# AUTOMATIC1111/stable-diffusion-webui

Measured on NVIDIA H100. Metric: images/sec SD1.5 txt2img 512x512, 20 Euler-a steps, batch 8 per GPU, higher is better.
Workload: dtype bf16

## Files before the change

### stable-diffusion-webui_b200/csrc/common.cuh

```cuda
#pragma once
#include <cuda.h>
#include <cuda_runtime.h>
#include <cuda_fp16.h>
#include <cuda_bf16.h>
#include <stdint.h>
#include <cstdio>
#include <cstring>

namespace sdxe {

enum : int { DT_F16 = 0, DT_BF16 = 1, DT_F32 = 2 };

#define SDXE_DEVINL __device__ __forceinline__

SDXE_DEVINL uint32_t smem_u32(const void* p) { return (uint32_t)__cvta_generic_to_shared(p); }
SDXE_DEVINL uint32_t lane_id() { return threadIdx.x & 31; }

SDXE_DEVINL bool elect_one() {
  uint32_t pred = 0;
  asm volatile(
      "{\n\t.reg .b32 rx;\n\t.reg .pred px;\n\t"
      "elect.sync rx|px, 0xffffffff;\n\t"
      "selp.b32 %0, 1, 0, px;\n\t}\n"
      : "=r"(pred));
  return pred != 0;
}

SDXE_DEVINL void mbar_init(uint32_t bar, uint32_t count) {
  asm volatile("mbarrier.init.shared::cta.b64 [%0], %1;" ::"r"(bar), "r"(count) : "memory");
}
SDXE_DEVINL void fence_mbar_init() { asm volatile("fence.mbarrier_init.release.cluster;" ::: "memory"); }
SDXE_DEVINL void mbar_expect_tx(uint32_t bar, uint32_t bytes) {
  asm volatile("mbarrier.arrive.expect_tx.shared::cta.b64 _, [%0], %1;" ::"r"(bar), "r"(bytes) : "memory");
}
SDXE_DEVINL void mbar_arrive(uint32_t bar) {
  asm volatile("mbarrier.arrive.shared::cta.b64 _, [%0];" ::"r"(bar) : "memory");
}
SDXE_DEVINL uint64_t global_timer_ns() {
  uint64_t t;
  asm volatile("mov.u64 %0, %%globaltimer;" : "=l"(t));
  return t;
}
SDXE_DEVINL void mbar_wait(uint32_t bar, uint32_t parity) {
  uint32_t done = 0;
  uint64_t t0 = 0;
  for (uint32_t it = 0;; ++it) {
    asm volatile(
        "{\n\t.reg .pred p;\n\t"
        "mbarrier.try_wait.parity.shared::cta.b64 p, [%1], %2;\n\t"
        "selp.b32 %0, 1, 0, p;\n\t}\n"
        : "=r"(done)
        : "r"(bar), "r"(parity)
        : "memory");
    if (done) return;
    if ((it & 0x3ff) == 0x3ff) {
      uint64_t now = global_timer_ns();
      if (t0 == 0) t0 = now;
      else if (now - t0 > 4000000000ull) __trap();
    }
  }
}

SDXE_DEVINL void pdl_launch_dependents() { asm volatile("griddepcontrol.launch_dependents;" ::: "memory"); }
SDXE_DEVINL void pdl_wait() { asm volatile("griddepcontrol.wait;" ::: "memory"); }

SDXE_DEVINL bool mbar_test(uint32_t bar, uint32_t parity) {
  uint32_t done;
  asm volatile(
      "{\n\t.reg .pred p;\n\t"
      "mbarrier.test_wait.parity.shared::cta.b64 p, [%1], %2;\n\t"
      "selp.b32 %0, 1, 0, p;\n\t}\n"
      : "=r"(done)
      : "r"(bar), "r"(parity)
      : "memory");
  return done != 0;
}

SDXE_DEVINL void fence_proxy_async_smem() { asm volatile("fence.proxy.async.shared::cta;" ::: "memory"); }

SDXE_DEVINL void tma_prefetch_desc(const CUtensorMap* m) {
  asm volatile("prefetch.tensormap [%0];" ::"l"(reinterpret_cast<uint64_t>(m)) : "memory");
}
SDXE_DEVINL void tma_load_2d(uint32_t dst, const CUtensorMap* m, uint32_t bar, int c0, int c1) {
  asm volatile(
      "cp.async.bulk.tensor.2d.shared::cluster.global.mbarrier::complete_tx::bytes [%0], [%1, {%3, %4}], [%2];"
      ::"r"(dst), "l"(reinterpret_cast<uint64_t>(m)), "r"(bar), "r"(c0), "r"(c1)
      : "memory");
}
SDXE_DEVINL void tma_load_3d(uint32_t dst, const CUtensorMap* m, uint32_t bar, int c0, int c1, int c2) {
  asm volatile(
      "cp.async.bulk.tensor.3d.shared::cluster.global.mbarrier::complete_tx::bytes [%0], [%1, {%3, %4, %5}], [%2];"
      ::"r"(dst), "l"(reinterpret_cast<uint64_t>(m)), "r"(bar), "r"(c0), "r"(c1), "r"(c2)
      : "memory");
}
SDXE_DEVINL void tma_load_4d(uint32_t dst, const CUtensorMap* m, uint32_t bar, int c0, int c1, int c2, int c3) {
  asm volatile(
      "cp.async.bulk.tensor.4d.shared::cluster.global.mbarrier::complete_tx::bytes [%0], [%1, {%3, %4, %5, %6}], [%2];"
      ::"r"(dst), "l"(reinterpret_cast<uint64_t>(m)), "r"(bar), "r"(c0), "r"(c1), "r"(c2), "r"(c3)
      : "memory");
}
SDXE_DEVINL void tma_load_5d(uint32_t dst, const CUtensorMap* m, uint32_t bar, int c0, int c1, int c2, int c3, int c4) {
  asm volatile(
      "cp.async.bulk.tensor.5d.shared::cluster.global.mbarrier::complete_tx::bytes [%0], [%1, {%3, %4, %5, %6, %7}], [%2];"
      ::"r"(dst), "l"(reinterpret_cast<uint64_t>(m)), "r"(bar), "r"(c0), "r"(c1), "r"(c2), "r"(c3), "r"(c4)
      : "memory");
}

SDXE_DEVINL void tma_store_2d(const CUtensorMap* m, uint32_t src, int c0, int c1) {
  asm volatile("cp.async.bulk.tensor.2d.global.shared::cta.bulk_group [%0, {%2, %3}], [%1];"
               ::"l"(reinterpret_cast<uint64_t>(m)), "r"(src), "r"(c0), "r"(c1)
               : "memory");
}
SDXE_DEVINL void bulk_commit_group() { asm volatile("cp.async.bulk.commit_group;" ::: "memory"); }
SDXE_DEVINL void bulk_wait_read_all() { asm volatile("cp.async.bulk.wait_group.read 0;" ::: "memory"); }
SDXE_DEVINL void bulk_wait_read_1() { asm volatile("cp.async.bulk.wait_group.read 1;" ::: "memory"); }
SDXE_DEVINL void bulk_wait_all() { asm volatile("cp.async.bulk.wait_group 0;" ::: "memory"); }

SDXE_DEVINL void wgmma_fence() { asm volatile("wgmma.fence.sync.aligned;" ::: "memory"); }
SDXE_DEVINL void wgmma_commit() { asm volatile("wgmma.commit_group.sync.aligned;" ::: "memory"); }
template <int N> SDXE_DEVINL void wgmma_wait() { asm volatile("wgmma.wait_group.sync.aligned %0;" ::"n"(N) : "memory"); }
SDXE_DEVINL void reg_fence(float& r) { asm volatile("" : "+f"(r)::"memory"); }

SDXE_DEVINL uint64_t gmma_desc_sw128(uint32_t saddr, uint32_t lbo_bytes, uint32_t sbo_bytes) {
  uint64_t d = 0;
  d |= (uint64_t)((saddr >> 4) & 0x3fff);
  d |= (uint64_t)((lbo_bytes >> 4) & 0x3fff) << 16;
  d |= (uint64_t)((sbo_bytes >> 4) & 0x3fff) << 32;
  d |= (uint64_t)1 << 62;
  return d;
}

template <bool BF16> struct T16;
template <> struct T16<false> {
  using type = __half;
  using type2 = __half2;
  static SDXE_DEVINL uint32_t pack(float a, float b) {
    __half2 h = __floats2half2_rn(a, b);
    return *reinterpret_cast<uint32_t*>(&h);
  }
  static SDXE_DEVINL float2 unpack(uint32_t u) { return __half22float2(*reinterpret_cast<__half2*>(&u)); }
  static SDXE_DEVINL float to_f(type v) { return __half2float(v); }
  static SDXE_DEVINL type from_f(float v) { return __float2half_rn(v); }
};
template <> struct T16<true> {
  using type = __nv_bfloat16;
  using type2 = __nv_bfloat162;
  static SDXE_DEVINL uint32_t pack(float a, float b) {
    __nv_bfloat162 h = __floats2bfloat162_rn(a, b);
    return *reinterpret_cast<uint32_t*>(&h);
  }
  static SDXE_DEVINL float2 unpack(uint32_t u) { return __bfloat1622float2(*reinterpret_cast<__nv_bfloat162*>(&u)); }
  static SDXE_DEVINL float to_f(type v) { return __bfloat162float(v); }
  static SDXE_DEVINL type from_f(float v) { return __float2bfloat16_rn(v); }
};

SDXE_DEVINL float ex2_approx(float x) {
  float y;
  asm("ex2.approx.ftz.f32 %0, %1;" : "=f"(y) : "f"(x));
  return y;
}
SDXE_DEVINL float ex2_poly3(float x) {
  x = fmaxf(x, -125.f);
  const float magic = 12582912.f;
  const float t = x + magic;
  const float r = x - (t - magic);
  float p = fmaf(0.0551716685295105f, r, 0.2426111400127411f);
  p = fmaf(p, r, 0.6932609677314758f);
  p = fmaf(p, r, 0.9999280571937561f);
  return __int_as_float(__float_as_int(p) + (__float_as_int(t) << 23));
}
SDXE_DEVINL float rcp_approx(float x) {
  float y;
  asm("rcp.approx.ftz.f32 %0, %1;" : "=f"(y) : "f"(x));
  return y;
}
SDXE_DEVINL float silu_f(float x) { return x * rcp_approx(1.f + ex2_approx(-1.4426950408889634f * x)); }
SDXE_DEVINL float gelu_erf_f(float x) { return 0.5f * x * (1.f + erff(x * 0.70710678118654752f)); }
#ifndef SDXE_GELU_V1
SDXE_DEVINL float gelu_fast_f(float x) {
  constexpr float C = 0.84932180028801904f;
  constexpr float S = 0.83255461115769776f;
  constexpr float H = 0.58870501125773735f;
  const float u = x * C;
  const float a = fabsf(u);
  const float t = rcp_approx(fmaf(0.3275911f * S, a, 1.f));
  float p = fmaf(1.061405429f * H, t, -1.453152027f * H);
  p = fmaf(p, t, 1.421413741f * H);
  p = fmaf(p, t, -0.284496736f * H);
  p = fmaf(p, t, 0.254829592f * H);
  const float e = ex2_approx(-u * u);
  return fmaf(-(a * e), p * t, fmaxf(x, 0.f));
}
#else
SDXE_DEVINL float gelu_fast_f(float x) {
  const float z = fabsf(x) * 0.70710678118654752f;
  const float t = rcp_approx(fmaf(0.3275911f, z, 1.f));
  float p = fmaf(1.061405429f, t, -1.453152027f);
  p = fmaf(p, t, 1.421413741f);
  p = fmaf(p, t, -0.284496736f);
  p = fmaf(p, t, 0.254829592f);
  const float e = ex2_approx(-z * z * 1.4426950408889634f);
  const float erf_abs = fmaf(-p * t, e, 1.f);
  const float erfv = copysignf(erf_abs, x);
  return 0.5f * x * (1.f + erfv);
}
#endif

#define SDXE_CUDA_CHECK(expr)                                                         \
  do {                                                                                \
    cudaError_t _e = (expr);                                                          \
    if (_e != cudaSuccess) {                                                          \
      ::sdxe::set_last_error(__FILE__, __LINE__, cudaGetErrorString(_e));             \
      return -1;                                                                      \
    }                                                                                 \
  } while (0)

void set_last_error(const char* file, int line, const char* msg);
const char* last_error();

int make_tmap_2d(CUtensorMap* out, const void* base, int64_t rows, int64_t cols, int64_t ld, int box_rows);
int make_tmap_2d_box(CUtensorMap* out, const void* base, int64_t rows, int64_t cols, int64_t ld, int box_cols, int box_rows);
int make_tmap_heads(CUtensorMap* out, const void* base, int64_t d, int64_t tokens, int64_t heads, int64_t batch,
                    int64_t tok_stride, int64_t head_stride, int64_t batch_stride, int box_rows);
int make_tmap_3d(CUtensorMap* out, const void* base, int64_t d0, int64_t d1, int64_t d2, int64_t pitch1, int64_t pitch2,
                 int box_rows);
int make_tmap_nhwc(CUtensorMap* out, const void* base, int N, int H, int W, int C, int bw, int bh, int bn);
int make_tmap_nhwc_s2(CUtensorMap* out, const void* base, int N, int H, int W, int C, int bw, int bh, int bn);

int num_sms();
bool pdl_enabled();

template <typename... KArgs, typename... Args>
inline cudaError_t launch_k(void (*kern)(KArgs...), dim3 grid, dim3 block, size_t smem, cudaStream_t s, Args&&... args) {
  cudaLaunchConfig_t cfg;
  memset(&cfg, 0, sizeof(cfg));
  cfg.gridDim = grid;
  cfg.blockDim = block;
  cfg.dynamicSmemBytes = smem;
  cfg.stream = s;
  cudaLaunchAttribute attr[1];
  attr[0].id = cudaLaunchAttributeProgrammaticStreamSerialization;
  attr[0].val.programmaticStreamSerializationAllowed = 1;
  cfg.attrs = attr;
  cfg.numAttrs = pdl_enabled() ? 1 : 0;
  return cudaLaunchKernelEx(&cfg, kern, static_cast<KArgs>(args)...);
}

}
```

### stable-diffusion-webui_b200/csrc/gemm.cu

```cuda
#include "gemm.cuh"
#include "wgmma.cuh"
#include <algorithm>
#include <cstdio>
#include <cstdlib>
#include <cstring>
#include <utility>

namespace sdxe {

static constexpr int BLOCK_M = 128;
static constexpr int BLOCK_K = 64;
static constexpr int A_STAGE_BYTES = BLOCK_M * BLOCK_K * 2;
static constexpr int GEMM_THREADS = 288;
static constexpr int CONSUMER_WARPS = 8;
static constexpr int SMEM_BUDGET = 227 * 1024;

template <int BN, bool BF16>
__global__ void __launch_bounds__(GEMM_THREADS, 1) gemm_kernel(const __grid_constant__ GemmArgs a) {
  using T = T16<BF16>;
  pdl_launch_dependents();
  extern __shared__ uint8_t smem_raw[];
  const uint32_t raw = smem_u32(smem_raw);
  const uint32_t smem_base = (raw + 1023u) & ~1023u;

  const int S = a.num_stages;
  constexpr uint32_t stage_bytes = A_STAGE_BYTES + BN * 128;
  const uint32_t bar_base = smem_base + S * stage_bytes;
  auto full_bar = [&](int s) { return bar_base + 8u * s; };
  auto empty_bar = [&](int s) { return bar_base + 8u * (S + s); };

  const int warp = threadIdx.x >> 5;
  const int lane = threadIdx.x & 31;
  const int num_m = (a.M + BLOCK_M - 1) / BLOCK_M;
  const int num_n = (a.N + BN - 1) / BN;
  const int num_kb = (a.K + BLOCK_K - 1) / BLOCK_K;
  const int num_tiles = num_m * num_n;

  if (threadIdx.x == 0) {
    for (int s = 0; s < S; ++s) {
      mbar_init(full_bar(s), 1);
      mbar_init(empty_bar(s), CONSUMER_WARPS);
    }
    fence_mbar_init();
    tma_prefetch_desc(&a.tmA);
    tma_prefetch_desc(&a.tmB);
  }
  __syncthreads();
  pdl_wait();

  if (warp == CONSUMER_WARPS) {
    int stage = 0;
    uint32_t phase = 0;
    for (int tile = blockIdx.x; tile < num_tiles; tile += gridDim.x) {
      const int n_blk = tile % num_n;
      const int m0 = (tile / num_n) * BLOCK_M;
      int img0 = 0, h0 = 0, w0 = 0;
      if (a.conv) {
        const int hw = a.H * a.W;
        img0 = m0 / hw;
        const int rem = m0 - img0 * hw;
        h0 = rem / a.W;
        w0 = rem - h0 * a.W;
      }
      int tap = 0, cb = 0;
      for (int kb = 0; kb < num_kb; ++kb) {
        mbar_wait(empty_bar(stage), phase ^ 1u);
        if (elect_one()) {
          const uint32_t sA = smem_base + stage * stage_bytes;
          const uint32_t sB = sA + A_STAGE_BYTES;
          const uint32_t fb = full_bar(stage);
          mbar_expect_tx(fb, stage_bytes);
          if (a.conv == 2) {
            const int dy = tap / 3, dx = tap - dy * 3;
            const int ty = dy - a.pad_lo, tx = dx - a.pad_lo;
            tma_load_5d(sA, &a.tmA, fb, (tx & 1) * (a.cblocks * BLOCK_K) + cb * BLOCK_K, w0 + (tx >> 1), ty & 1, h0 + (ty >> 1), img0);
          } else if (a.conv) {
            const int dy = tap / 3, dx = tap - dy * 3;
            tma_load_4d(sA, &a.tmA, fb, cb * BLOCK_K, w0 + dx - 1, h0 + dy - 1, img0);
          } else {
            const int k0 = kb * BLOCK_K;
            if (k0 < a.K1) tma_load_2d(sA, &a.tmA, fb, k0, m0);
            else tma_load_2d(sA, &a.tmA2, fb, k0 - a.K1, m0);
          }
          tma_load_2d(sB, &a.tmB, fb, kb * BLOCK_K, n_blk * BN);
        }
        __syncwarp();
        if (++cb == a.cblocks) { cb = 0; ++tap; }
        if (++stage == S) { stage = 0; phase ^= 1u; }
      }
    }
    return;
  }

  const int wg = warp >> 2;
  const int band = (warp & 3) * 16 + (lane >> 2);
  const int cq = 2 * (lane & 3);
  const int M = a.M, N = a.N;
  const uint64_t adesc0 = gmma_desc_sw128(smem_base + (uint32_t)wg * (64 * 128), 16, 1024);
  const uint64_t bdesc0 = gmma_desc_sw128(smem_base + A_STAGE_BYTES, 16, 1024);
  constexpr uint32_t stage_inc = stage_bytes >> 4;
  float acc[BN / 2];
  int stage = 0;
  uint32_t phase = 0;
  for (int tile = blockIdx.x; tile < num_tiles; tile += gridDim.x) {
    const int n_blk = tile % num_n;
    const int m_blk = tile / num_n;
    int prev = -1;
    for (int kb = 0; kb < num_kb; ++kb) {
      mbar_wait(full_bar(stage), phase);
      wgmma_fence();
      const uint64_t ad = adesc0 + (uint64_t)(stage * stage_inc);
      const uint64_t bd = bdesc0 + (uint64_t)(stage * stage_inc);
      wgmma_ss<BN, BF16>(acc, ad, bd, kb != 0);
      wgmma_ss<BN, BF16>(acc, ad + 2, bd + 2, 1);
      wgmma_ss<BN, BF16>(acc, ad + 4, bd + 4, 1);
      wgmma_ss<BN, BF16>(acc, ad + 6, bd + 6, 1);
      wgmma_commit();
      if (prev >= 0) {
        wgmma_wait<1>();
        if (lane == 0) mbar_arrive(empty_bar(prev));
      }
      prev = stage;
      if (++stage == S) { stage = 0; phase ^= 1u; }
    }
    wgmma_wait<0>();
#pragma unroll
    for (int i = 0; i < BN / 2; ++i) reg_fence(acc[i]);
    if (lane == 0 && prev >= 0) mbar_arrive(empty_bar(prev));

    const int row0 = m_blk * BLOCK_M + wg * 64 + band;
    float ln_mu[2] = {0.f, 0.f}, ln_rs[2] = {1.f, 1.f};
    if (a.c1) {
#pragma unroll
      for (int h = 0; h < 2; ++h) {
        const int m = row0 + 8 * h;
        float ps = 0.f, pq = 0.f;
        if (m < M) {
          for (int pp = 0; pp < a.ln_parts; ++pp) {
            const float2 t = __ldg(a.ln_part + (size_t)pp * M + m);
            ps += t.x;
            pq += t.y;
          }
        }
        ln_mu[h] = ps * a.ln_inv_c;
        ln_rs[h] = rsqrtf(fmaxf(pq * a.ln_inv_c - ln_mu[h] * ln_mu[h], 0.f) + a.ln_eps);
      }
    }
    if (a.epi == EPI_GEGLU) {
      constexpr int HALF = BN / 2;
      const int ldo = a.ldo;
#pragma unroll
      for (int i = 0; i < HALF / 8; ++i) {
        const int jl = 8 * i + cq;
        const int cv = n_blk * BN + jl, cg = cv + HALF;
        float bv[2] = {0.f, 0.f}, bg[2] = {0.f, 0.f}, kv[2] = {0.f, 0.f}, kg[2] = {0.f, 0.f};
        if (a.bias) { bv[0] = __ldg(a.bias + cv); bv[1] = __ldg(a.bias + cv + 1); bg[0] = __ldg(a.bias + cg); bg[1] = __ldg(a.bias + cg + 1); }
        if (a.c1) { kv[0] = __ldg(a.c1 + cv); kv[1] = __ldg(a.c1 + cv + 1); kg[0] = __ldg(a.c1 + cg); kg[1] = __ldg(a.c1 + cg + 1); }
#pragma unroll
        for (int h = 0; h < 2; ++h) {
          const int m = row0 + 8 * h;
          float o[2];
#pragma unroll
          for (int e = 0; e < 2; ++e) {
            float v = acc[4 * i + 2 * h + e], g = acc[4 * (i + HALF / 8) + 2 * h + e];
            if (a.c1) {
              v = fmaf(ln_rs[h], v - ln_mu[h] * kv[e], bv[e]);
              g = fmaf(ln_rs[h], g - ln_mu[h] * kg[e], bg[e]);
            } else {
              v += bv[e];
              g += bg[e];
            }
            o[e] = v * gelu_fast_f(g);
          }
          if (m < M) *reinterpret_cast<uint32_t*>(reinterpret_cast<uint16_t*>(a.out) + (size_t)m * ldo + n_blk * HALF + jl) = T::pack(o[0], o[1]);
        }
      }
    } else {
      const int n_store = std::min((N + 7) / 8 * 8, a.ldo);
      const int n_res = a.residual ? std::min((N + 7) / 8 * 8, a.ldr) : 0;
      const float* rv[2] = {nullptr, nullptr};
      bool row_ok[2];
#pragma unroll
      for (int h = 0; h < 2; ++h) {
        const int m = row0 + 8 * h;
        row_ok[h] = m < M;
        if (a.rowvec && row_ok[h]) rv[h] = a.rowvec + (size_t)(m / a.rows_per_sample) * a.ldrv;
      }
      float st_s[2] = {0.f, 0.f}, st_q[2] = {0.f, 0.f};
#pragma unroll
      for (int i = 0; i < BN / 8; ++i) {
        const int col = n_blk * BN + 8 * i + cq;
        if (col >= n_store) continue;
        const bool in0 = col < N, in1 = col + 1 < N;
        float b[2] = {0.f, 0.f}, k[2] = {0.f, 0.f};
        if (a.bias) { b[0] = in0 ? __ldg(a.bias + col) : 0.f; b[1] = in1 ? __ldg(a.bias + col + 1) : 0.f; }
        if (a.c1) { k[0] = in0 ? __ldg(a.c1 + col) : 0.f; k[1] = in1 ? __ldg(a.c1 + col + 1) : 0.f; }
#pragma unroll
        for (int h = 0; h < 2; ++h) {
          if (!row_ok[h]) continue;
          const size_t m = (size_t)(row0 + 8 * h);
          float v0 = acc[4 * i + 2 * h], v1 = acc[4 * i + 2 * h + 1];
          if (a.c1) {
            v0 = fmaf(ln_rs[h], v0 - ln_mu[h] * k[0], b[0]);
            v1 = fmaf(ln_rs[h], v1 - ln_mu[h] * k[1], b[1]);
          } else {
            v0 += b[0];
            v1 += b[1];
          }
          if (rv[h]) {
            if (in0) v0 += __ldg(rv[h] + col);
            if (in1) v1 += __ldg(rv[h] + col + 1);
          }
          if (col < n_res) {
            const uint32_t r = __ldg(reinterpret_cast<const unsigned int*>(reinterpret_cast<const uint16_t*>(a.residual) + m * a.ldr + col));
            const float2 f = T::unpack(r);
            v0 += f.x;
            v1 += f.y;
          }
          const uint32_t pk = T::pack(v0, v1);
          *reinterpret_cast<uint32_t*>(reinterpret_cast<uint16_t*>(a.out) + m * a.ldo + col) = pk;
          if (a.stat_out) {
            const float2 f = T::unpack(pk);
            const float x0 = in0 ? f.x : 0.f, x1 = in1 ? f.y : 0.f;
            st_s[h] += x0 + x1;
            st_q[h] = fmaf(x0, x0, fmaf(x1, x1, st_q[h]));
          }
        }
      }
      if (a.stat_out) {
#pragma unroll
        for (int h = 0; h < 2; ++h) {
          st_s[h] += __shfl_xor_sync(0xffffffffu, st_s[h], 1);
          st_q[h] += __shfl_xor_sync(0xffffffffu, st_q[h], 1);
          st_s[h] += __shfl_xor_sync(0xffffffffu, st_s[h], 2);
          st_q[h] += __shfl_xor_sync(0xffffffffu, st_q[h], 2);
          if ((lane & 3) == 0 && row_ok[h]) a.stat_out[(size_t)n_blk * M + row0 + 8 * h] = make_float2(st_s[h], st_q[h]);
        }
      }
    }
  }
}

bool conv_tile_shape(int H, int W, int* bw, int* bh, int* bn) {
  if (W >= 128) {
    if (W % 128) return false;
    *bw = 128; *bh = 1; *bn = 1;
    return true;
  }
  if (128 % W) return false;
  const int rows = 128 / W;
  if (H >= rows) {
    if (H % rows) return false;
    *bw = W; *bh = rows; *bn = 1;
    return true;
  }
  if (rows % H) return false;
  *bw = W; *bh = H; *bn = rows / H;
  return true;
}

static size_t gemm_smem_fixed(int num_stages) {
  return 1024  + 16 * (size_t)num_stages;
}
static size_t gemm_smem(int BN, int num_stages) { return (size_t)num_stages * (A_STAGE_BYTES + BN * 128) + gemm_smem_fixed(num_stages); }

int gemm_pick_stages(int BN) {
  const int stage_bytes = A_STAGE_BYTES + BN * 128;
  const int s = (int)((SMEM_BUDGET - gemm_smem_fixed(8)) / stage_bytes);
  return std::max(2, std::min(s, 8));
}

int gemm_finish_args(GemmArgs& a, const void* W, int64_t w_rows, int64_t w_ld) {
  a.num_stages = gemm_pick_stages(a.BN);
  if (a.ldo % 8 || (a.residual && a.ldr % 8)) { set_last_error(__FILE__, __LINE__, "gemm: ldo / ldr must be multiples of 8"); return -1; }
  return make_tmap_2d(&a.tmB, W, w_rows, a.K, w_ld, a.BN);
}

int gemm_pick_bn(int M, int N, int K, int epi) {
  (void)K;
  const int sms = num_sms();
  const int num_m = (M + BLOCK_M - 1) / BLOCK_M;
  double best = 1e30;
  int best_bn = 16;
  for (int bn = 16; bn <= 256; bn += 16) {
    if (epi == EPI_GEGLU && (bn % 32 != 0 || N % bn != 0)) continue;
    const int num_n = (N + bn - 1) / bn;
    const long tiles = (long)num_m * num_n;
    const long waves = (tiles + sms - 1) / sms;
    const double kb = std::max(4.0 * bn, (A_STAGE_BYTES + 128.0 * bn) / 32.0) + 64.0;
    const double cost = waves * kb;
    if (cost < best - 1e-9) { best = cost; best_bn = bn; }
  }
  return best_bn;
}

typedef void (*GemmKernel)(const GemmArgs);
static constexpr int GEMM_NUM_BN = 16;
template <std::size_t... I>
static GemmKernel gemm_variant_impl(int i, bool bf16, std::index_sequence<I...>) {
  static const GemmKernel k16[] = {gemm_kernel<16 * (int)(I + 1), false>...};
  static const GemmKernel kb16[] = {gemm_kernel<16 * (int)(I + 1), true>...};
  return bf16 ? kb16[i] : k16[i];
}
static GemmKernel gemm_variant(int BN, bool bf16) {
  return gemm_variant_impl(BN / 16 - 1, bf16, std::make_index_sequence<GEMM_NUM_BN>{});
}

int gemm_init() {
  static bool done = false;
  if (!done) {
    for (int bn = 16; bn <= 256; bn += 16)
      for (int b = 0; b < 2; ++b)
        SDXE_CUDA_CHECK(cudaFuncSetAttribute(gemm_variant(bn, b != 0), cudaFuncAttributeMaxDynamicSharedMemorySize, SMEM_BUDGET));
    done = true;
  }
  return 0;
}

int gemm_launch(const GemmArgs& a, bool bf16, cudaStream_t stream) {
  if (a.BN % 16 != 0 || a.BN < 16 || a.BN > 256) { set_last_error(__FILE__, __LINE__, "gemm: bad BN"); return -1; }
  if (a.K1 != a.K && (a.K1 % BLOCK_K) != 0) { set_last_error(__FILE__, __LINE__, "gemm: K1 % 64"); return -1; }
  if (a.epi == EPI_GEGLU && (a.BN % 32 != 0 || a.N % a.BN != 0)) { set_last_error(__FILE__, __LINE__, "gemm: geglu tile"); return -1; }
  if ((a.epi != EPI_PLAIN) && (a.residual || a.rowvec || a.stat_out)) { set_last_error(__FILE__, __LINE__, "gemm: residual / rowvec / statistics need EPI_PLAIN"); return -1; }
  if ((a.c1 && (a.residual || a.stat_out || a.rowvec)) || (a.stat_out && a.rowvec)) {
    set_last_error(__FILE__, __LINE__, "gemm: unsupported LayerNorm-fold / statistics combination");
    return -1;
  }
  if (a.num_stages < 2) { set_last_error(__FILE__, __LINE__, "gemm: stages (call gemm_finish_args)"); return -1; }
  const size_t smem = gemm_smem(a.BN, a.num_stages);
  if (smem > (size_t)SMEM_BUDGET) { set_last_error(__FILE__, __LINE__, "gemm: shared memory budget"); return -1; }
  const int num_m = (a.M + BLOCK_M - 1) / BLOCK_M, num_n = (a.N + a.BN - 1) / a.BN;
  const int tiles = num_m * num_n;
  if (tiles <= 0) return 0;
  if (gemm_init() != 0) return -1;
  const int grid = std::min(tiles, num_sms());
  SDXE_CUDA_CHECK(launch_k(gemm_variant(a.BN, bf16), dim3(grid), dim3(GEMM_THREADS), smem, stream, a));
  SDXE_CUDA_CHECK(cudaGetLastError());
  return 0;
}

}
```

Before: 8.499.

## Rebalance registers via setmaxnreg and batch epilogue loads in groups

Raises the block size to 384 threads (a full producer warpgroup) so setmaxnreg can move registers from producer warps (40) to consumer warps (232), and the three spare producer warps exit early. Separately, the GEMM epilogue now issues bias, LN-coefficient, row-vector and residual loads for groups of four column blocks before doing the arithmetic, so global-load latency overlaps instead of serializing per column. The intent is to ease register pressure from the large accumulator and hide epilogue load latency. The cost is more live registers in the epilogue and a dependency on setmaxnreg constraints, which require warpgroup-aligned launches and enough registers in the launch_bounds budget.

```diff
diff --git a/stable-diffusion-webui_b200/csrc/common.cuh b/stable-diffusion-webui_b200/csrc/common.cuh
--- a/stable-diffusion-webui_b200/csrc/common.cuh
+++ b/stable-diffusion-webui_b200/csrc/common.cuh
@@ -120,6 +120,9 @@
 SDXE_DEVINL void wgmma_commit() { asm volatile("wgmma.commit_group.sync.aligned;" ::: "memory"); }
 template <int N> SDXE_DEVINL void wgmma_wait() { asm volatile("wgmma.wait_group.sync.aligned %0;" ::"n"(N) : "memory"); }
 SDXE_DEVINL void reg_fence(float& r) { asm volatile("" : "+f"(r)::"memory"); }
+
+template <int N> SDXE_DEVINL void setmaxnreg_dec() { asm volatile("setmaxnreg.dec.sync.aligned.u32 %0;" ::"n"(N)); }
+template <int N> SDXE_DEVINL void setmaxnreg_inc() { asm volatile("setmaxnreg.inc.sync.aligned.u32 %0;" ::"n"(N)); }
 
 SDXE_DEVINL uint64_t gmma_desc_sw128(uint32_t saddr, uint32_t lbo_bytes, uint32_t sbo_bytes) {
   uint64_t d = 0;
diff --git a/stable-diffusion-webui_b200/csrc/gemm.cu b/stable-diffusion-webui_b200/csrc/gemm.cu
--- a/stable-diffusion-webui_b200/csrc/gemm.cu
+++ b/stable-diffusion-webui_b200/csrc/gemm.cu
@@ -11,8 +11,11 @@
 static constexpr int BLOCK_M = 128;
 static constexpr int BLOCK_K = 64;
 static constexpr int A_STAGE_BYTES = BLOCK_M * BLOCK_K * 2;
-static constexpr int GEMM_THREADS = 288;
+static constexpr int GEMM_THREADS = 384;
 static constexpr int CONSUMER_WARPS = 8;
+static constexpr int PRODUCER_REGS = 40;
+static constexpr int CONSUMER_REGS = 232;
+static constexpr int EPI_GROUPS = 4;
 static constexpr int SMEM_BUDGET = 227 * 1024;
 
 template <int BN, bool BF16>
@@ -48,7 +51,9 @@
   __syncthreads();
   pdl_wait();
 
-  if (warp == CONSUMER_WARPS) {
+  if (warp >= CONSUMER_WARPS) {
+    setmaxnreg_dec<PRODUCER_REGS>();
+    if (warp != CONSUMER_WARPS) return;
     int stage = 0;
     uint32_t phase = 0;
     for (int tile = blockIdx.x; tile < num_tiles; tile += gridDim.x) {
@@ -92,6 +97,7 @@
     return;
   }
 
+  setmaxnreg_inc<CONSUMER_REGS>();
   const int wg = warp >> 2;
   const int band = (warp & 3) * 16 + (lane >> 2);
   const int cq = 2 * (lane & 3);
@@ -150,80 +156,111 @@
       constexpr int HALF = BN / 2;
       const int ldo = a.ldo;
 #pragma unroll
-      for (int i = 0; i < HALF / 8; ++i) {
-        const int jl = 8 * i + cq;
-        const int cv = n_blk * BN + jl, cg = cv + HALF;
-        float bv[2] = {0.f, 0.f}, bg[2] = {0.f, 0.f}, kv[2] = {0.f, 0.f}, kg[2] = {0.f, 0.f};
-        if (a.bias) { bv[0] = __ldg(a.bias + cv); bv[1] = __ldg(a.bias + cv + 1); bg[0] = __ldg(a.bias + cg); bg[1] = __ldg(a.bias + cg + 1); }
-        if (a.c1) { kv[0] = __ldg(a.c1 + cv); kv[1] = __ldg(a.c1 + cv + 1); kg[0] = __ldg(a.c1 + cg); kg[1] = __ldg(a.c1 + cg + 1); }
-#pragma unroll
-        for (int h = 0; h < 2; ++h) {
-          const int m = row0 + 8 * h;
-          float o[2];
+      for (int i0 = 0; i0 < HALF / 8; i0 += EPI_GROUPS) {
+        float bv[EPI_GROUPS][2], bg[EPI_GROUPS][2], kv[EPI_GROUPS][2], kg[EPI_GROUPS][2];
+#pragma unroll
+        for (int g = 0; g < EPI_GROUPS && i0 + g < HALF / 8; ++g) {
+          const int cv = n_blk * BN + 8 * (i0 + g) + cq, cg = cv + HALF;
 #pragma unroll
           for (int e = 0; e < 2; ++e) {
-            float v = acc[4 * i + 2 * h + e], g = acc[4 * (i + HALF / 8) + 2 * h + e];
-            if (a.c1) {
-              v = fmaf(ln_rs[h], v - ln_mu[h] * kv[e], bv[e]);
-              g = fmaf(ln_rs[h], g - ln_mu[h] * kg[e], bg[e]);
-            } else {
-              v += bv[e];
-              g += bg[e];
-            }
-            o[e] = v * gelu_fast_f(g);
-          }
-          if (m < M) *reinterpret_cast<uint32_t*>(reinterpret_cast<uint16_t*>(a.out) + (size_t)m * ldo + n_blk * HALF + jl) = T::pack(o[0], o[1]);
+            bv[g][e] = a.bias ? __ldg(a.bias + cv + e) : 0.f;
+            bg[g][e] = a.bias ? __ldg(a.bias + cg + e) : 0.f;
+            kv[g][e] = a.c1 ? __ldg(a.c1 + cv + e) : 0.f;
+            kg[g][e] = a.c1 ? __ldg(a.c1 + cg + e) : 0.f;
+          }
+        }
+#pragma unroll
+        for (int g = 0; g < EPI_GROUPS && i0 + g < HALF / 8; ++g) {
+          const int i = i0 + g;
+          const int jl = 8 * i + cq;
+#pragma unroll
+          for (int h = 0; h < 2; ++h) {
+            const int m = row0 + 8 * h;
+            float o[2];
+#pragma unroll
+            for (int e = 0; e < 2; ++e) {
+              float v = acc[4 * i + 2 * h + e], gt = acc[4 * (i + HALF / 8) + 2 * h + e];
+              if (a.c1) {
+                v = fmaf(ln_rs[h], v - ln_mu[h] * kv[g][e], bv[g][e]);
+                gt = fmaf(ln_rs[h], gt - ln_mu[h] * kg[g][e], bg[g][e]);
+              } else {
+                v += bv[g][e];
+                gt += bg[g][e];
+              }
+              o[e] = v * gelu_fast_f(gt);
+            }
+            if (m < M) *reinterpret_cast<uint32_t*>(reinterpret_cast<uint16_t*>(a.out) + (size_t)m * ldo + n_blk * HALF + jl) = T::pack(o[0], o[1]);
+          }
         }
       }
     } else {
       const int n_store = std::min((N + 7) / 8 * 8, a.ldo);
       const int n_res = a.residual ? std::min((N + 7) / 8 * 8, a.ldr) : 0;
       const float* rv[2] = {nullptr, nullptr};
+      const uint16_t* rres[2] = {nullptr, nullptr};
       bool row_ok[2];
 #pragma unroll
       for (int h = 0; h < 2; ++h) {
         const int m = row0 + 8 * h;
         row_ok[h] = m < M;
         if (a.rowvec && row_ok[h]) rv[h] = a.rowvec + (size_t)(m / a.rows_per_sample) * a.ldrv;
+        if (a.residual && row_ok[h]) rres[h] = reinterpret_cast<const uint16_t*>(a.residual) + (size_t)m * a.ldr;
       }
       float st_s[2] = {0.f, 0.f}, st_q[2] = {0.f, 0.f};
 #pragma unroll
-      for (int i = 0; i < BN / 8; ++i) {
-        const int col = n_blk * BN + 8 * i + cq;
-        if (col >= n_store) continue;
-        const bool in0 = col < N, in1 = col + 1 < N;
-        float b[2] = {0.f, 0.f}, k[2] = {0.f, 0.f};
-        if (a.bias) { b[0] = in0 ? __ldg(a.bias + col) : 0.f; b[1] = in1 ? __ldg(a.bias + col + 1) : 0.f; }
-        if (a.c1) { k[0] = in0 ? __ldg(a.c1 + col) : 0.f; k[1] = in1 ? __ldg(a.c1 + col + 1) : 0.f; }
-#pragma unroll
-        for (int h = 0; h < 2; ++h) {
-          if (!row_ok[h]) continue;
-          const size_t m = (size_t)(row0 + 8 * h);
-          float v0 = acc[4 * i + 2 * h], v1 = acc[4 * i + 2 * h + 1];
-          if (a.c1) {
-            v0 = fmaf(ln_rs[h], v0 - ln_mu[h] * k[0], b[0]);
-            v1 = fmaf(ln_rs[h], v1 - ln_mu[h] * k[1], b[1]);
-          } else {
-            v0 += b[0];
-            v1 += b[1];
-          }
-          if (rv[h]) {
-            if (in0) v0 += __ldg(rv[h] + col);
-            if (in1) v1 += __ldg(rv[h] + col + 1);
-          }
-          if (col < n_res) {
-            const uint32_t r = __ldg(reinterpret_cast<const unsigned int*>(reinterpret_cast<const uint16_t*>(a.residual) + m * a.ldr + col));
-            const float2 f = T::unpack(r);
-            v0 += f.x;
-            v1 += f.y;
-          }
-          const uint32_t pk = T::pack(v0, v1);
-          *reinterpret_cast<uint32_t*>(reinterpret_cast<uint16_t*>(a.out) + m * a.ldo + col) = pk;
-          if (a.stat_out) {
-            const float2 f = T::unpack(pk);
-            const float x0 = in0 ? f.x : 0.f, x1 = in1 ? f.y : 0.f;
-            st_s[h] += x0 + x1;
-            st_q[h] = fmaf(x0, x0, fmaf(x1, x1, st_q[h]));
+      for (int i0 = 0; i0 < BN / 8; i0 += EPI_GROUPS) {
+        float b[EPI_GROUPS][2], k[EPI_GROUPS][2], r[EPI_GROUPS][2][2];
+        uint32_t res[EPI_GROUPS][2];
+#pragma unroll
+        for (int g = 0; g < EPI_GROUPS && i0 + g < BN / 8; ++g) {
+          const int col = n_blk * BN + 8 * (i0 + g) + cq;
+          const bool in0 = col < N, in1 = col + 1 < N;
+          b[g][0] = a.bias && in0 ? __ldg(a.bias + col) : 0.f;
+          b[g][1] = a.bias && in1 ? __ldg(a.bias + col + 1) : 0.f;
+          k[g][0] = a.c1 && in0 ? __ldg(a.c1 + col) : 0.f;
+          k[g][1] = a.c1 && in1 ? __ldg(a.c1 + col + 1) : 0.f;
+#pragma unroll
+          for (int h = 0; h < 2; ++h) {
+            r[g][h][0] = rv[h] && in0 ? __ldg(rv[h] + col) : 0.f;
+            r[g][h][1] = rv[h] && in1 ? __ldg(rv[h] + col + 1) : 0.f;
+            res[g][h] = rres[h] && col < n_res ? __ldg(reinterpret_cast<const unsigned int*>(rres[h] + col)) : 0u;
+          }
+        }
+#pragma unroll
+        for (int g = 0; g < EPI_GROUPS && i0 + g < BN / 8; ++g) {
+          const int i = i0 + g;
+          const int col = n_blk * BN + 8 * i + cq;
+          if (col >= n_store) continue;
+          const bool in0 = col < N, in1 = col + 1 < N;
+#pragma unroll
+          for (int h = 0; h < 2; ++h) {
+            if (!row_ok[h]) continue;
+            const size_t m = (size_t)(row0 + 8 * h);
+            float v0 = acc[4 * i + 2 * h], v1 = acc[4 * i + 2 * h + 1];
+            if (a.c1) {
+              v0 = fmaf(ln_rs[h], v0 - ln_mu[h] * k[g][0], b[g][0]);
+              v1 = fmaf(ln_rs[h], v1 - ln_mu[h] * k[g][1], b[g][1]);
+            } else {
+              v0 += b[g][0];
+              v1 += b[g][1];
+            }
+            if (rv[h]) {
+              if (in0) v0 += r[g][h][0];
+              if (in1) v1 += r[g][h][1];
+            }
+            if (col < n_res) {
+              const float2 f = T::unpack(res[g][h]);
+              v0 += f.x;
+              v1 += f.y;
+            }
+            const uint32_t pk = T::pack(v0, v1);
+            *reinterpret_cast<uint32_t*>(reinterpret_cast<uint16_t*>(a.out) + m * a.ldo + col) = pk;
+            if (a.stat_out) {
+              const float2 f = T::unpack(pk);
+              const float x0 = in0 ? f.x : 0.f, x1 = in1 ? f.y : 0.f;
+              st_s[h] += x0 + x1;
+              st_q[h] = fmaf(x0, x0, fmaf(x1, x1, st_q[h]));
+            }
           }
         }
       }
```

After: 9.667 (median of 6 runs). 1.14x the previous value.
